# lsalzman/enet

Measured on AMD Instinct MI355X. Metric: GiB/s device-resident range-coder (de)compress, 64Ki×1200B pkts, 1/2/4/8 GPU, higher is better.
Workload: dtype u8; 1 GPU; C2 65536x1200B uniform-random, compress+decompress round trip; packets_per_gpu=65536, packet_bytes=1200, parallelism=shard1, out_cap=2N+64

## Files before the change

enet_amd/csrc/rc_dec6.hip:

```cpp


#ifndef RC_LANE_HOST_TEST
#include <hip/hip_runtime.h>
#else
#include "lane_host_shim.h"
#endif
#include <stdint.h>
#include <type_traits>

#include "rc_abi_internal.h"
#include "rc_udiv.h"
#include "rc_lane_common.h"
#include "rc_root3.h"
#include "rc_dec6_rare.h"
#include "rc_slot.h"

namespace {

#ifndef DEC6_BLOCK
#define DEC6_BLOCK 16
#endif
#ifndef DEC6_PRIO
#define DEC6_PRIO 3
#endif
#ifndef DEC6_HELP_SLEEP
#define DEC6_HELP_SLEEP 4
#endif
#ifndef DEC6_RARE_ITERS
#define DEC6_RARE_ITERS 2
#endif
constexpr uint32_t kBlock6 = DEC6_BLOCK;
constexpr uint32_t kRareIters6 = DEC6_RARE_ITERS;
constexpr uint32_t kWaveBail6 = 16;
constexpr uint32_t kStats6 = kRootStrideDec;
constexpr uint32_t kLds6 = kRootStrideDec + 256;
constexpr uint32_t kDummy6 = 256 * kTab2Rec;

DEV void bail6(const rc_workspace_dev& ws, uint32_t pkt) { bail(ws, pkt); }

DEV void reset6(uint8_t* root, uint8_t* stats, Root& R, uint32_t& rtot, double& rrt, uint32_t& order, uint32_t& a,
                uint32_t& p, uint32_t& nodes, uint32_t& nh, bool& repeat, bool& o2s, bool& e2d, uint32_t& seg0,
                uint32_t& rst, uint32_t n)
{
    root3_clear<false>(root, R);
    const uint4 z = make_uint4(0u, 0u, 0u, 0u);
#pragma unroll
    for (int i = 0; i < 16; ++i) reinterpret_cast<uint4*>(stats)[i] = z;
    rtot = 1 + 256;
    rrt = rcp64(rtot);
    order = 0; a = 0; p = 0; nodes = 1; nh = 0;
    repeat = false; o2s = false; e2d = false;
    rst = (rst | (n << (12 * (rst >> 24)))) + (1u << 24);
    seg0 = n;
}

DEV bool can_reset6(uint32_t rst, uint32_t n) { return (rst >> 24) < 2 && n < 4096; }

struct ByteSink1 {
    uint32_t acc, nb, ws;
    uint4 w, wp;
    bool pend;
    uintptr_t waddr, wpaddr, lo;
    uint32_t n, cap;
};

DEV void sink1_init(ByteSink1& o, uint8_t* p, uint32_t cap)
{
    o.lo = reinterpret_cast<uintptr_t>(p);
    o.waddr = o.lo & ~static_cast<uintptr_t>(15);
    o.wpaddr = o.waddr;
    o.ws = static_cast<uint32_t>(o.lo & 15) >> 2;
    o.nb = static_cast<uint32_t>(o.lo & 3);
    o.acc = 0;
    o.w = make_uint4(0u, 0u, 0u, 0u);
    o.wp = o.w;
    o.pend = false;
    o.n = 0;
    o.cap = cap;
}

DEV void sink1_flush(ByteSink1& o)
{
    sink_store(o.wpaddr, o.wp, o.lo, o.pend);
    o.pend = false;
}

DEV void sink1_put(ByteSink1& o, uint32_t v, bool en)
{
    o.acc |= en ? (v << (8 * o.nb)) : 0u;
    o.nb += en ? 1u : 0u;
    o.n += en ? 1u : 0u;
    const bool mv = o.nb == 4;
    o.w.x = mv ? o.w.y : o.w.x; o.w.y = mv ? o.w.z : o.w.y; o.w.z = mv ? o.w.w : o.w.z; o.w.w = mv ? o.acc : o.w.w;
    o.acc = mv ? 0u : o.acc;
    o.nb = mv ? 0u : o.nb;
    o.ws += mv ? 1u : 0u;
    const bool full = o.ws == 4;
    o.wp.x = full ? o.w.x : o.wp.x; o.wp.y = full ? o.w.y : o.wp.y;
    o.wp.z = full ? o.w.z : o.wp.z; o.wp.w = full ? o.w.w : o.wp.w;
    o.wpaddr = full ? o.waddr : o.wpaddr;
    o.pend = o.pend || full;
    o.ws = full ? 0u : o.ws;
    o.waddr += full ? 16 : 0;
}

DEV void sink1_finish(ByteSink1& o)
{
    sink1_flush(o);
    const uint32_t ws = o.ws;
    const uint32_t d[4] = {o.w.x, o.w.y, o.w.z, o.w.w};
    uint32_t q[4];
#pragma unroll
    for (uint32_t j = 0; j < 4; ++j) {
        const uint32_t k = 4 - ws + j;
        q[j] = j < ws ? (k == 0 ? d[0] : k == 1 ? d[1] : k == 2 ? d[2] : d[3]) : (j == ws ? o.acc : 0u);
    }
    sink_bytes(o.waddr, make_uint4(q[0], q[1], q[2], q[3]), 0ull, 4 * ws + o.nb, o.lo);
}

template <class Src>
DEV void decompress_one6(const rc_batch_dev& bt, const rc_workspace_dev& ws, uint32_t pkt, uint8_t* root,
                         uint8_t* stats, uint8_t* tab, uint8_t* tab2, const uint8_t* itab, Src& in,
                         const double* rtab = nullptr)
{
    constexpr bool kSlot = std::is_same<Src, SlotSrc>::value;
    const uint32_t len = bt.in_len[pkt];
    const uint32_t cap = bt.out_cap[pkt];
    if (len == 0) { bt.out_len[pkt] = 0; ws.claims[pkt] = 0; ws.dec6_resets[pkt] = 0; return; }
    ByteSink1 o;
    sink1_init(o, bt.out + bt.out_off[pkt], cap);
    uint32_t code;
    if constexpr (kSlot) {
        code = slot_init(in, bt.in + bt.in_off[pkt], len, pkt);
    } else {
        src_init(in, bt.in + bt.in_off[pkt], len);
        code = static_cast<uint32_t>(in.la >> 32);
        in.la <<= 32;
        in.na -= 4;
        src_refill(in, true);
    }
    Root R;
    root3_clear<false>(root, R);
    {
        const uint4 z = make_uint4(0u, 0u, 0u, 0u);
#pragma unroll
        for (int i = 0; i < 16; ++i) reinterpret_cast<uint4*>(stats)[i] = z;
    }
    uint32_t rtot = 1 + 256;
    double rrt = rcp64(rtot);
    uint32_t low = 0, range = ~0u;

    uint32_t order = 0, a = 0, p = 0, nodes = 1, claims = 0, x0 = 0;
    uint32_t hl[4] = {0u, 0u, 0u, 0u}, nh = 0;
    bool repeat = false;
    bool o2s = false;
    bool e2d = false;
    bool stall = false, done = false, off = false, fail = false;
    uint32_t seg0 = 0, rst = 0;

    PROF_DECL
    uint32_t s = 0;
#ifdef DEC6_STATS_PREFETCH
    uint32_t stn = 0;
    double rtn = 1.0;
#endif
    for (;;) {
        {
            uint32_t shc = 0;
            uint4 ssl = make_uint4(0u, 0u, 0u, 0u);
            if constexpr (kSlot) {
                slot_read(in, shc, ssl);
            } else {
                src_fill(in, true);
            }
            sink1_flush(o);
            const bool go = !done && !stall;
#ifdef DEC6_STATS_PREFETCH
            const uint32_t st = (go && order >= 1) ? stn : 0u;
#else
            const uint32_t sraw = stats[p];
            const uint32_t st = (go && order >= 1) ? sraw : 0u;
#endif
            const uint32_t t1 = st & 31u, d1 = t1 - (st >> 5);
            bool need = go && order >= 2 && repeat && !o2s;
            bool e2 = false;
            const bool c2s = go && order >= 2 && repeat && o2s;
            if (any_lane(c2s)) {
                const uint32_t r2 = udiv16d(range, 7u, 1.0 / 7.0);
                e2 = c2s && code - low < 5u * r2;
                need = need || (c2s && !e2);
                range = e2 ? r2 : range;
                dec_code(low, code, range, 0u, 5u, in, e2);
            }
            const bool o1 = go && !need && order >= 1 && t1 > 0;
            const uint32_t esc1 = kSubEscDelta * d1, tot1 = o1 ? esc1 + kSubDelta * t1 : 1u;
#ifdef DEC6_STATS_PREFETCH
            const uint32_t r1 = udiv16d(range, tot1, o1 ? rtn : 1.0);
#elif defined(DEC6_RCP_TAB) && !defined(RC_LANE_HOST_TEST)
            const uint32_t r1 = udiv16d(range, tot1, rtab[st]);
#else
            const uint32_t r1 = udiv16d(range, tot1, rcp64(tot1));
#endif
#ifndef DEC6_READ1
            const bool e1 = o1 && code - low < esc1 * r1;
            need = need || (o1 && !e1);
#else
            const uint32_t cd1 = udiv_lo16(code - low, r1);
            need = need || (o1 && cd1 >= esc1);
            const bool e1 = o1 && cd1 < esc1;
#endif
            need = need && !(ws.dec6_debug & 2);
            range = e1 ? r1 : range;
            dec_code(low, code, range, 0u, esc1, in, e1);
            const bool rg = go && !need;
            const uint32_t r0 = udiv16d(range, rtot, rrt);
            const uint32_t cd0 = udiv_lo16(code - low, r0);
            const bool eos = rg && cd0 < 1;
            const bool past = rg && !eos && cd0 - 1 >= rtot - 1;
            const bool sym = rg && !eos && !past;
            range = sym ? r0 : range;
            uint32_t under0 = 0, cnt0 = 0;
#ifndef DEC6_ITAB_LATE
            uint4 i0, i1;
            const uint32_t v = root3_search_inc(root, R, itab, sym ? cd0 - 1 : 0u, under0, cnt0, i0, i1);
#else
            const uint32_t v = root3_search(root, R, sym ? cd0 - 1 : 0u, under0, cnt0);
#endif
            dec_code_late(low, code, range, 1 + under0, 1 + cnt0, in, sym);
            if (sym) {
#ifndef DEC6_ITAB_LATE
                root3_add_pre(root, R, v, cnt0, i0, i1);
#else
                root3_add_inc(root, R, itab, v, cnt0);
#endif
                rtot = (rtot + kRootDelta) & 0xFFFF;
            }
            if (rare_lane(sym && (1 + cnt0 > 0xFF - 2 * kRootDelta + 1 || rtot > kTotalLimit))) {
                if (sym && (1 + cnt0 > 0xFF - 2 * kRootDelta + 1 || rtot > kTotalLimit))
                    rtot = root3_rescale<false>(root, R);
            }
            rrt = sym ? rcp64(rtot) : rrt;
            nodes += sym ? (cnt0 == 0 ? 1u : 0u) + (order >= 1 ? 1u : 0u) + (order >= 2 ? 1u : 0u) : 0u;
            const bool o1v = sym && order >= 1;
#ifndef DEC6_STATS_PREFETCH
            stats[p] = static_cast<uint8_t>(o1v ? st + 1 : sraw);
#else
            if (o1v) stats[p] = static_cast<uint8_t>(st + 1);
#endif
            const bool full = o1v && t1 >= kTabCap;
            *GPTR(uint16_t, !(o1v && !full) ? reinterpret_cast<uintptr_t>(tab2) + kDummy6 : rec_addr(tab, tab2, p, t1)) =
                static_cast<uint16_t>(a | (v << 8));
            x0 = (sym && order == 0) ? v : x0;
            const bool fl = sym && o.n >= o.cap;
            claims += (o1v && !fl) ? 1u : 0u;
            const bool rs0 = sym && nodes >= kMaxNodes;
            const bool lv = past || full || (rs0 && !can_reset6(rst, o.n + 1));
            off = off || lv;
            fail = fail || fl;
            done = done || eos || lv || fl;
            sink1_put(o, v, sym && !lv && !fl);
            a = sym ? p : a;
            p = sym ? v : p;
            order += (sym && order < 2) ? 1u : 0u;
            repeat = sym ? false : repeat;
            o2s = sym ? false : o2s;
            e2d = go ? (e2 && need) : e2d;
            stall = stall || need;
            if (rare_lane(rs0 && !done)) {
                if (rs0 && !done) reset6(root, stats, R, rtot, rrt, order, a, p, nodes, nh, repeat, o2s, e2d, seg0, rst, o.n);
            }
#ifdef DEC6_STATS_PREFETCH
            stn = stats[p];
            {
                const uint32_t nt = stn & 31u, nd1 = nt - (stn >> 5);
                rtn = rcp64(max(kSubEscDelta * nd1 + kSubDelta * nt, 1u));
            }
#endif
            PROF(0)
            if constexpr (kSlot) slot_step_end(in, ssl, shc);
            else src_adv(in);
            PROF(5)
        }
        ++s;
        if (s < kBlock6 && any_lane(!done && !stall)) continue;
        s = 0;
        for (uint32_t it = 0; it < kRareIters6 && any_lane(stall && !done); ++it) {
            const bool rs = stall && !done;
            uint32_t shc = 0;
            uint4 ssl = make_uint4(0u, 0u, 0u, 0u);
            if constexpr (kSlot) {
                slot_read(in, shc, ssl);
            } else {
                src_fill(in, true);
            }
            sink1_flush(o);
#ifdef DEC6_DRAIN
            __builtin_amdgcn_s_waitcnt(0);
#endif
            const uint32_t st = rs && order >= 1 ? stats[p] : 0u;
            const uint32_t t1 = st & 31u, d1 = t1 - (st >> 5);
            Hist6 H;
            rec_build(tab, tab2, p, rs ? t1 : 0u, hl, nh, x0, o.n - seg0, rs, H);
            const bool over = false;
            PROF(1)
#ifdef RC_PROFILE
            prof_acc[8] += 1;
            prof_acc[9] += static_cast<unsigned long long>(__builtin_popcountll(__builtin_amdgcn_ballot_w64(rs)));
#endif
            uint32_t nd = 1;
#pragma unroll
            for (uint32_t j = 1; j < 8; ++j) nd += any_lane(H.k > 4 * j) ? 1u : 0u;
            uint32_t pl[8];
            planes6(H.V, nd, pl);
            const uint32_t km = low_bits(H.k);
            const uint32_t g2 = (rs && order >= 2) ? (eqmask6(H.A, a, nd) & km & ~H.p1) : 0u;
            const uint32_t g1 = km & ~H.hit;
            const uint32_t t2 = popc(g2);
            uint32_t d2 = 0;
            {
                uint32_t rem = g2;
                while (any_lane(rem != 0)) {
                    const uint32_t j = rem ? static_cast<uint32_t>(__builtin_ctz(rem)) : 0u;
                    const uint32_t same = peq6(pl, pval6(pl, j)) & g2 & low_bits(j);
                    d2 += (rem != 0 && same == 0) ? 1u : 0u;
                    rem &= rem ? rem - 1u : 0u;
                }
            }
            int at = -1;
            uint32_t v = 0, hu = 0, hc = 0;
            bool sf = false;
            const bool c2 = rs && !over && !e2d && order >= 2 && t2 > 0;
            if (any_lane(c2)) {
                if (sub_decode6(pl, g2, t2, d2, c2, low, code, range, in, v, hu, hc, sf)) at = 2;
            }
            const bool c1 = rs && !over && !sf && at < 0 && order >= 1 && t1 > 0;
            if (any_lane(c1)) {
                if (sub_decode6(pl, g1, t1, d1, c1, low, code, range, in, v, hu, hc, sf)) at = 1;
            }
            const bool rg = rs && !over && !sf && at < 0;
            const uint32_t r0 = udiv16d(range, rtot, rrt);
            const uint32_t cd0 = udiv_lo16(code - low, r0);
            const bool eos = rg && cd0 < 1;
            const bool past = rg && !eos && cd0 - 1 >= rtot - 1;
            const bool sym0 = rg && !eos && !past;
            range = sym0 ? r0 : range;
            uint32_t under0 = 0, cnt0 = 0;
            const uint32_t v0 = root3_search(root, R, sym0 ? cd0 - 1 : 0u, under0, cnt0);
            const bool sym = sym0 || at > 0;
            v = sym0 ? v0 : v;
            dec_code(low, code, range, sym0 ? 1 + under0 : hu, sym0 ? 1 + cnt0 : hc, in, sym);
            if (sym0) {
                root3_add_inc(root, R, itab, v, cnt0);
                rtot = (rtot + kRootDelta) & 0xFFFF;
            }
            if (rare_lane(sym0 && (1 + cnt0 > 0xFF - 2 * kRootDelta + 1 || rtot > kTotalLimit))) {
                if (sym0 && (1 + cnt0 > 0xFF - 2 * kRootDelta + 1 || rtot > kTotalLimit))
                    rtot = root3_rescale<false>(root, R);
            }
            rrt = sym0 ? rcp64(rtot) : rrt;
            PROF(2)
            const uint32_t eqv = peq6(pl, v) & km;
            const bool n2 = order >= 2 && (eqv & g2) == 0;
            const bool n1 = order >= 1 && at != 2 && (eqv & g1) == 0;
            const bool nb = eqv == 0;
            nodes += sym ? (sym0 && cnt0 == 0 ? 1u : 0u) + (n2 ? 1u : 0u) + (n1 ? 1u : 0u) : 0u;
            const bool o1v = sym && order >= 1 && at != 2;
            const uint32_t nst = st + 1 + (n1 ? 0u : 32u);
            if (o1v) stats[p] = static_cast<uint8_t>(nst);
            const bool tfull = o1v && t1 >= kTabCap;
            if (o1v && !tfull)
                *GPTR(uint16_t, rec_addr(tab, tab2, p, t1)) =
                    static_cast<uint16_t>(a | (v << 8));
            claims += (sym && order >= 1 && nb && o.n < o.cap) ? 1u : 0u;
            const bool h2 = sym && at == 2;
            const uint32_t he = p | (a << 8) | (v << 16);
#pragma unroll
            for (uint32_t h = 0; h < 4; ++h) hl[h] = (h2 && nh == h) ? he : hl[h];
            const bool hfull = h2 && nh >= 4;
            nh += h2 ? 1u : 0u;
            const bool fl = sym && o.n >= o.cap;
            const bool rs0 = rs && sym && nodes >= kMaxNodes;
            const bool lv = over || sf || past || hfull || tfull || (o1v && !n1 && (st >> 5) >= 7) ||
                            (rs0 && !can_reset6(rst, o.n + 1));
            off = off || (rs && lv);
            fail = fail || (rs && fl);
            done = done || (rs && (eos || lv || fl));
            sink1_put(o, v, sym && !lv && !fl);
            a = sym ? p : a;
            p = sym ? v : p;
            order += (sym && order < 2) ? 1u : 0u;
            repeat = sym ? !nb : repeat;
            const bool one = sym && popc(eqv) == 1;
            o2s = rs ? one : o2s;
            e2d = rs ? false : e2d;
            stall = rs ? (sym && !lv && !fl && order >= 2 && repeat && !one) : stall;
            if (rare_lane(rs0 && !done)) {
                if (rs0 && !done) {
                    reset6(root, stats, R, rtot, rrt, order, a, p, nodes, nh, repeat, o2s, e2d, seg0, rst, o.n);
                    stall = false;
                }
            }
            if constexpr (kSlot) slot_step_end(in, ssl, shc);
            else src_adv(in);
            PROF(3)
        }
#ifdef DEC6_END_WAIT
        __builtin_amdgcn_s_waitcnt(0);
#endif
#ifdef DEC6_STATS_PREFETCH
        stn = stats[p];
        {
            const uint32_t nt = stn & 31u, nd1 = nt - (stn >> 5);
            rtn = rcp64(max(kSubEscDelta * nd1 + kSubDelta * nt, 1u));
        }
#endif
        const uint32_t left = static_cast<uint32_t>(__builtin_popcountll(__builtin_amdgcn_ballot_w64(off)));
        if (left >= kWaveBail6) { off = off || !done; done = true; }
        PROF(4)
        if (!any_lane(!done)) break;
    }
    PROF_FLUSH(16)
#ifndef DEC6_NO_USED_CHECK
    if constexpr (kSlot) {
        const uint32_t used = 16 * in.j + 4 * in.q - in.lo15 - in.na;
        off = off || (!fail && (used < len || used > len + 4));
    }
#endif
    if (off) { bail6(ws, pkt); ws.claims[pkt] = 0xFFFFFFFFu; return; }
    ws.dec6_resets[pkt] = rst;
    if constexpr (kSlot) ws.dec6_icks[pkt] = in.cks;
    sink1_finish(o);
    bt.out_len[pkt] = o.n;
    ws.claims[pkt] = claims | (fail ? 0x80000000u : 0u);
}

}

#ifndef RC_LANE_HOST_TEST
constexpr uint32_t kLanes6s = 256;
extern "C" __global__ __launch_bounds__(512) void rc_decompress_dec6s(rc_batch_dev b, rc_workspace_dev ws)
{
    extern __shared__ __attribute__((aligned(16))) uint8_t smem[];
    const uint32_t wave = threadIdx.x >> 6;
    const bool helper = wave >= 4;
    const uint32_t L = (wave & 3) * 64 + (threadIdx.x & 63);
    uint8_t* root = smem + L * kLds6;
    uint8_t* stats = root + kStats6;
    uint8_t* slotp = root + 256;
    uint32_t* mctl = reinterpret_cast<uint32_t*>(smem + kLanes6s * kLds6) + 2 * L;
    uint32_t* hctl = reinterpret_cast<uint32_t*>(smem + kLanes6s * kLds6 + 8 * kLanes6s) + L;
    uint8_t* itab = smem + kLanes6s * (kLds6 + 12);
    const uint32_t slot = blockIdx.x * kLanes6s + L;
    if (!helper) *reinterpret_cast<uint2*>(mctl) = make_uint2(0u, slot < b.n ? kNoPktS : kFinS);
    else *hctl = 0u;
    if (threadIdx.x < 16) root3_inc_init(itab, threadIdx.x);
    double* rtab = reinterpret_cast<double*>(itab + 512);
#ifdef DEC6_RCP_TAB
    if (threadIdx.x < 256) {
        const uint32_t t1 = threadIdx.x & 31u, r1 = threadIdx.x >> 5;
        const uint32_t tot = (t1 > 0 && r1 <= t1) ? kSubEscDelta * (t1 - r1) + kSubDelta * t1 : 1u;
        rtab[threadIdx.x] = rcp64(tot);
    }
#endif
    __syncthreads();
    if (helper) {
        SlotHelp h;
        slot_help_init(h);
#ifdef DEC6_HELP_COUNT
        uint32_t nb = 0, ni = 0;
#endif
        for (;;) {
            bool fin = false;
            const bool busy = slot_help_iter(b, mctl, hctl, slotp, h, ws.dec6_hcks, ws.n_cap, fin);
#ifdef DEC6_HELP_COUNT
            nb += busy ? 1u : 0u;
            ni += busy ? 0u : 1u;
#endif
            if (fin) break;
            if (!busy) __builtin_amdgcn_s_sleep(DEC6_HELP_SLEEP);
        }
#ifdef DEC6_HELP_COUNT
        if ((threadIdx.x & 63) == 0) { atomicAdd(&ws.counters[5], nb); atomicAdd(&ws.counters[6], ni); }
#endif
        return;
    }
    uint8_t* tab = static_cast<uint8_t*>(ws.dec6_pool) + static_cast<size_t>(slot) * kTab1;
    uint8_t* tab2 = static_cast<uint8_t*>(ws.dec6_pool) + static_cast<size_t>(ws.lane_slots) * kTab1 +
                    static_cast<size_t>(slot) * kTab2;
    const uint32_t* order = ws.order && !ws.bins[RC_LEN_BINS] ? ws.order : nullptr;
    __builtin_amdgcn_s_setprio(DEC6_PRIO);
    SlotSrc in;
    in.gen = 0; in.mctl = mctl; in.hctl = hctl; in.slot = slotp;
    for (uint32_t i = slot; i < b.n; i += gridDim.x * kLanes6s) {
        const uint32_t pkt = order ? order[i] : i;
        decompress_one6(b, ws, pkt, root, stats, tab, tab2, itab, in, rtab);
    }
    mctl[1] = kFinS;
}

constexpr uint32_t kVerifyWaves = 4;
constexpr uint32_t kVerifyBlocksPerCu = 10;
constexpr uint32_t kVerDw = 8;

DEV uint32_t vhead_load(const rc_batch_dev& b, const rc_workspace_dev& ws, uint32_t k, uint32_t l)
{
    const uint32_t* src = l == 0 ? ws.claims + k
                        : l == 1 ? b.out_len + k
                        : l < 4 ? reinterpret_cast<const uint32_t*>(b.out_off + k) + (l - 2)
                        : l == 4 ? ws.dec6_resets + k
                        : l == 5 ? ws.dec6_icks + k
                        : l == 6 ? ws.dec6_hcks + k
                                 : ws.dec6_hcks + ws.n_cap + k;
    return (k < b.n && l < 8) ? *src : 0u;
}


struct VHead {
    uint32_t cl, n, rst, off, nd;
    uintptr_t lo, sb;
    bool skip, fast, cks;
};

DEV VHead vhead_get(const rc_batch_dev& b, uint32_t k, uint32_t hv)
{
    VHead h;
    h.cl = __shfl(hv, 0);
    h.n = __shfl(hv, 1);
    const uint64_t oo = static_cast<uint64_t>(static_cast<uint32_t>(__shfl(hv, 2))) |
                        static_cast<uint64_t>(static_cast<uint32_t>(__shfl(hv, 3))) << 32;
    h.rst = __shfl(hv, 4);
    h.cks = cks_agree(__shfl(hv, 5), __shfl(hv, 6), __shfl(hv, 7));
    h.skip = k >= b.n || h.cl == 0xFFFFFFFFu;
    h.lo = reinterpret_cast<uintptr_t>(b.out) + oo;
    h.sb = h.lo & ~static_cast<uintptr_t>(3);
    h.off = static_cast<uint32_t>(h.lo - h.sb);
    h.nd = (h.off + h.n + 3) >> 2;
    h.fast = !h.skip && (h.rst >> 24) == 0 && h.nd <= 64 * kVerDw;
    return h;
}

DEV void vdata_load(const VHead& h, uint32_t l, uint32_t (&w)[kVerDw])
{
    const uint32_t* p = reinterpret_cast<const uint32_t*>(h.sb);
#pragma unroll
    for (uint32_t r = 0; r < kVerDw; ++r) {
        const uint32_t c = 64 * r + l;
        w[r] = (h.fast && c < h.nd) ? p[c] : 0u;
    }
}

DEV void vresult(const rc_batch_dev& b, const rc_workspace_dev& ws, uint32_t k, uint32_t cl, uint32_t cnt, bool ck,
                 uint32_t l)
{
    for (int sft = 32; sft >= 1; sft >>= 1) cnt += static_cast<uint32_t>(__shfl_xor(static_cast<int>(cnt), sft));
    const uint32_t want = cl & 0x7FFFFFFFu;
    const bool ok = cnt == want && ck && !(ws.dec6_debug & 1);
    if (l == 0 && !ok) {
        const uint32_t i = atomicAdd(&ws.counters[3], 1u);
        ws.enc2_list[i] = k;
        if (!ck) atomicAdd(&ws.counters[7], 1u);
    }
    if (l == 0 && ok && (cl >> 31)) b.out_len[k] = 0;
}

DEV void vclear(uint4* set4, uint32_t l)
{
#pragma unroll
    for (uint32_t i = 0; i < 512 / 64; ++i) set4[i * 64 + l] = make_uint4(0u, 0u, 0u, 0u);
}

DEV void verify_fast(const rc_batch_dev& b, const rc_workspace_dev& ws, uint32_t k, const VHead& h,
                     const uint32_t (&w)[kVerDw], uint4* set4, uint32_t l)
{
    uint32_t* set = reinterpret_cast<uint32_t*>(set4);
    vclear(set4, l);
    uint32_t cnt = 0, last = 0;
#pragma unroll
    for (uint32_t r = 0; r < kVerDw; ++r) {
        if (64 * r >= h.nd) break;
        const uint32_t up = static_cast<uint32_t>(__shfl_up(static_cast<int>(w[r]), 1));
        const uint32_t pw = l ? up : last;
        last = static_cast<uint32_t>(__shfl(static_cast<int>(w[r]), 63));
        const uint32_t c = 64 * r + l;
#pragma unroll
        for (uint32_t t = 0; t < 4; ++t) {
            const uint32_t x = (w[r] >> (8 * t)) & 0xFFu;
            const uint32_t pv = t ? (w[r] >> (8 * t - 8)) & 0xFFu : pw >> 24;
            const uint32_t pos = 4 * c + t - h.off;
            const bool in = pos >= 1 && pos < h.n;
            const uint32_t bg = (pv << 8) | x, bit = 1u << (bg & 31);
#ifdef VERIFY_RETURNS
            const uint32_t old = atomicOr(&set[in ? bg >> 5 : l], in ? bit : 0u);
            cnt += (in && !(old & bit)) ? 1u : 0u;
#else
            atomicOr(&set[in ? bg >> 5 : l], in ? bit : 0u);
#endif
        }
    }
#ifndef VERIFY_RETURNS
    __builtin_amdgcn_fence(__ATOMIC_SEQ_CST, "wavefront");
    __builtin_amdgcn_wave_barrier();
#pragma unroll
    for (uint32_t i = 0; i < 512 / 64; ++i) {
        const uint4 q = set4[i * 64 + l];
        cnt += static_cast<uint32_t>(__builtin_popcount(q.x) + __builtin_popcount(q.y) + __builtin_popcount(q.z) +
                                     __builtin_popcount(q.w));
    }
#endif
    vresult(b, ws, k, h.cl, cnt, h.cks, l);
}

DEV void verify_slow(const rc_batch_dev& b, const rc_workspace_dev& ws, uint32_t pkt, uint4* set4, uint32_t l)
{
    uint32_t* set = reinterpret_cast<uint32_t*>(set4);
    {
        const uint32_t cl = ws.claims[pkt];
        const uint32_t n = b.out_len[pkt];
        const uintptr_t lo = reinterpret_cast<uintptr_t>(b.out + b.out_off[pkt]);
        const uint32_t rst = ws.dec6_resets[pkt], nseg = (rst >> 24) + 1;
        uint32_t cnt = 0;
        for (uint32_t sg = 0; sg < nseg; ++sg) {
            const uint32_t s0 = sg ? (rst >> (12 * (sg - 1))) & 0xFFFu : 0u;
            const uint32_t s1 = sg + 1 < nseg ? (rst >> (12 * sg)) & 0xFFFu : n;
#pragma unroll
            for (uint32_t i = 0; i < 512 / 64; ++i) set4[i * 64 + l] = make_uint4(0u, 0u, 0u, 0u);
            __builtin_amdgcn_wave_barrier();
            const uintptr_t slo = lo + s0;
            const uintptr_t sb = slo & ~static_cast<uintptr_t>(15);
            const uint32_t m = s1 > s0 ? s1 - s0 : 0u;
            const uint32_t chunks = m > 1 ? static_cast<uint32_t>((slo + m - sb + 15) >> 4) : 0u;
            for (uint32_t c = l; c < chunks; c += 64) {
                const uintptr_t a = sb + 16 * c;
                const uint4 w = *reinterpret_cast<const uint4*>(a);
                uint32_t prev = a > slo ? *reinterpret_cast<const uint8_t*>(a - 1) : 0u;
                const uint32_t d[4] = {w.x, w.y, w.z, w.w};
#pragma unroll
                for (uint32_t t = 0; t < 16; ++t) {
                    const uint32_t x = (d[t >> 2] >> (8 * (t & 3))) & 0xFFu;
                    const uintptr_t at = a + t;
                    if (at > slo && at < slo + m) {
                        const uint32_t bg = (prev << 8) | x;
                        atomicOr(&set[bg >> 5], 1u << (bg & 31));
                    }
                    prev = x;
                }
            }
            __builtin_amdgcn_wave_barrier();
            uint32_t sc = 0;
#pragma unroll
            for (uint32_t i = 0; i < 512 / 64; ++i) {
                const uint4 q = set4[i * 64 + l];
                sc += static_cast<uint32_t>(__builtin_popcount(q.x) + __builtin_popcount(q.y) +
                                            __builtin_popcount(q.z) + __builtin_popcount(q.w));
            }
            cnt += sc;
            __builtin_amdgcn_wave_barrier();
        }
        vresult(b, ws, pkt, cl, cnt, cks_agree(ws.dec6_icks[pkt], ws.dec6_hcks[pkt], ws.dec6_hcks[ws.n_cap + pkt]), l);
    }
}

DEV void verify_one(const rc_batch_dev& b, const rc_workspace_dev& ws, uint32_t k, const VHead& h,
                    const uint32_t (&w)[kVerDw], uint4* set4, uint32_t l)
{
    if (h.skip) return;
    if (h.fast) verify_fast(b, ws, k, h, w, set4, l);
    else verify_slow(b, ws, k, set4, l);
    __builtin_amdgcn_wave_barrier();
}

extern "C" __global__ __launch_bounds__(256) __attribute__((amdgpu_waves_per_eu(5)))
void rc_dec6_verify(rc_batch_dev b, rc_workspace_dev ws)
{
    __shared__ uint4 bits[kVerifyWaves][512];
    const uint32_t wave = threadIdx.x >> 6, l = threadIdx.x & 63;
    uint4* set4 = bits[wave];
    const uint32_t stride = gridDim.x * kVerifyWaves;
    uint32_t k = blockIdx.x * kVerifyWaves + wave;
    if (k >= b.n) return;
    uint32_t wa[kVerDw], wb[kVerDw];
    uint32_t hva = vhead_load(b, ws, k, l);
    VHead ha = vhead_get(b, k, hva), hb;
    vdata_load(ha, l, wa);
    uint32_t hvb = vhead_load(b, ws, k + stride, l);
    for (;;) {
        hb = vhead_get(b, k + stride, hvb);
        vdata_load(hb, l, wb);
        hva = vhead_load(b, ws, k + 2 * stride, l);
        verify_one(b, ws, k, ha, wa, set4, l);
        k += stride;
        if (k >= b.n) break;
        ha = vhead_get(b, k + stride, hva);
        vdata_load(ha, l, wa);
        hvb = vhead_load(b, ws, k + 2 * stride, l);
        verify_one(b, ws, k, hb, wb, set4, l);
        k += stride;
        if (k >= b.n) break;
    }
}

extern "C" int rc_hip_dec6_verify_launch(const rc_batch_dev* b, const rc_workspace_dev* ws, void* stream)
{
    hipStream_t st = static_cast<hipStream_t>(stream);
    const uint32_t vb = (b->n + kVerifyWaves - 1) / kVerifyWaves;
    static const char* vb_env = getenv("ENET_RC_VERIFY_BPC");
    const uint32_t bpc = vb_env && atoi(vb_env) > 0 ? static_cast<uint32_t>(atoi(vb_env)) : kVerifyBlocksPerCu;
    const uint32_t cap = (ws->cus ? ws->cus : 256u) * bpc;
    hipLaunchKernelGGL(rc_dec6_verify, dim3(vb < cap ? vb : cap), dim3(256), 0, st, *b, *ws);
    return static_cast<int>(hipGetLastError());
}

extern "C" int rc_hip_dec6_launch(const rc_batch_dev* b, const rc_workspace_dev* ws, uint32_t blocks, void* stream)
{
    hipStream_t st = static_cast<hipStream_t>(stream);
    if (ws->lane_active != 64) return static_cast<int>(hipErrorInvalidValue);
#ifdef DEC6_RCP_TAB
    const size_t lds = static_cast<size_t>(kLanes6s) * (kLds6 + 12) + 512 + 2048;
#else
    const size_t lds = static_cast<size_t>(kLanes6s) * (kLds6 + 12) + 512;
#endif
    hipLaunchKernelGGL(rc_decompress_dec6s, dim3(blocks), dim3(512), lds, st, *b, *ws);
    const hipError_t e = hipGetLastError();
    if (e != hipSuccess) return static_cast<int>(e);
    return rc_hip_dec6_verify_launch(b, ws, stream);
}
#endif
```

enet_amd/csrc/rc_dec6_rare.h:

```cpp
#pragma once

namespace {

DEV uint32_t eq01(uint32_t x, uint32_t y)
{
    const uint32_t z = x ^ y;
    const uint32_t t = ((z & 0x7F7F7F7Fu) + 0x7F7F7F7Fu) | z;
    return (~t >> 7) & 0x01010101u;
}

DEV uint32_t gather4(uint32_t e) { return (e | (e >> 7) | (e >> 14) | (e >> 21)) & 0xFu; }

DEV uint32_t popc(uint32_t x) { return static_cast<uint32_t>(__builtin_popcount(x)); }
DEV uint32_t low_bits(uint32_t n) { return n >= 32 ? 0xFFFFFFFFu : ((1u << n) - 1u); }

DEV void bail(const rc_workspace_dev& ws, uint32_t pkt)
{
    const uint32_t slot = atomicAdd(&ws.counters[3], 1u);
    ws.enc2_list[slot] = pkt;
}

constexpr uint32_t kTab1 = 256 * 16;
constexpr uint32_t kTab2Rec = 48;
constexpr uint32_t kTab2 = 256 * kTab2Rec + 128;
constexpr uint32_t kTabCap = 28;

struct Hist6 { uint32_t A[8], V[8]; uint32_t p1, hit, k; };

DEV uint4 hload16(uintptr_t a)
{
#ifndef RC_LANE_HOST_TEST
    const uint64_t lo = __hip_atomic_load(GPTRC(uint64_t, a), __ATOMIC_RELAXED, __HIP_MEMORY_SCOPE_AGENT);
    const uint64_t hi = __hip_atomic_load(GPTRC(uint64_t, a + 8), __ATOMIC_RELAXED, __HIP_MEMORY_SCOPE_AGENT);
    return make_uint4(static_cast<uint32_t>(lo), static_cast<uint32_t>(lo >> 32), static_cast<uint32_t>(hi),
                      static_cast<uint32_t>(hi >> 32));
#else
    return gload16(a);
#endif
}

DEV uint32_t eqmask6(const uint32_t* X, uint32_t u, uint32_t nd)
{
    const uint32_t ur = u * 0x01010101u;
    uint32_t m = 0;
#pragma unroll
    for (uint32_t d = 0; d < 8; ++d)
        if (d < nd) m |= gather4(eq01(X[d], ur)) << (4 * d);
    return m;
}

DEV uintptr_t rec_addr(const uint8_t* tab, const uint8_t* tab2, uint32_t p, uint32_t t)
{
    return t < 8 ? reinterpret_cast<uintptr_t>(tab) + 16 * p + 2 * t
                 : reinterpret_cast<uintptr_t>(tab2) + kTab2Rec * p + 2 * (t - 8);
}

DEV void rec_load(const uint8_t* tab, const uint8_t* tab2, uint32_t p, uint32_t t1, bool en, uint4& r1, uint4& r2,
                  uint4& r3, uint4& r4)
{
    const uint4 z = make_uint4(0u, 0u, 0u, 0u);
    r1 = z; r2 = z; r3 = z; r4 = z;
    const uintptr_t b2 = reinterpret_cast<uintptr_t>(tab2) + kTab2Rec * p;
    if (en) r1 = hload16(reinterpret_cast<uintptr_t>(tab) + 16 * p);
    if (en && t1 > 8) {
        r2 = hload16(b2);
        r3 = hload16(b2 + 16);
    }
    if (rare_lane(en && t1 > 24)) {
        if (en && t1 > 24) r4 = hload16(b2 + 32);
    }
}

DEV void rec_fill(const uint4& r1, const uint4& r2, const uint4& r3, const uint4& r4, uint32_t p, uint32_t t1,
                  const uint32_t* hl, uint32_t nh, uint32_t x0, uint32_t n, Hist6& H)
{
    H.A[0] = bperm(r1.y, r1.x, 0x06040200u); H.V[0] = bperm(r1.y, r1.x, 0x07050301u);
    H.A[1] = bperm(r1.w, r1.z, 0x06040200u); H.V[1] = bperm(r1.w, r1.z, 0x07050301u);
    H.A[2] = bperm(r2.y, r2.x, 0x06040200u); H.V[2] = bperm(r2.y, r2.x, 0x07050301u);
    H.A[3] = bperm(r2.w, r2.z, 0x06040200u); H.V[3] = bperm(r2.w, r2.z, 0x07050301u);
    H.A[4] = bperm(r3.y, r3.x, 0x06040200u); H.V[4] = bperm(r3.y, r3.x, 0x07050301u);
    H.A[5] = bperm(r3.w, r3.z, 0x06040200u); H.V[5] = bperm(r3.w, r3.z, 0x07050301u);
    H.A[6] = bperm(r4.y, r4.x, 0x06040200u); H.V[6] = bperm(r4.y, r4.x, 0x07050301u);
    H.A[7] = 0u; H.V[7] = 0u;
    H.p1 = (p == x0 && t1 > 0 && n >= 2) ? 1u : 0u;
    H.hit = 0u;
    uint32_t k = t1;
    if (any_lane(nh > 0))
#pragma unroll
    for (uint32_t h = 0; h < 4; ++h) {
        const bool mine = h < nh && (hl[h] & 0xFFu) == p;
        const uint32_t ks = 8 * (k & 3);
#pragma unroll
        for (uint32_t d = 0; d < 8; ++d) {
            const bool here = mine && (k >> 2) == d;
            H.A[d] = here ? ((H.A[d] & ~(0xFFu << ks)) | (((hl[h] >> 8) & 0xFFu) << ks)) : H.A[d];
            H.V[d] = here ? ((H.V[d] & ~(0xFFu << ks)) | (((hl[h] >> 16) & 0xFFu) << ks)) : H.V[d];
        }
        H.hit |= mine ? (1u << k) : 0u;
        k += mine ? 1u : 0u;
    }
    H.k = k;
}

DEV void rec_build(const uint8_t* tab, const uint8_t* tab2, uint32_t p, uint32_t t1, const uint32_t* hl, uint32_t nh,
                   uint32_t x0, uint32_t n, bool en, Hist6& H)
{
    uint4 r1, r2, r3, r4;
    rec_load(tab, tab2, p, t1, en, r1, r2, r3, r4);
    rec_fill(r1, r2, r3, r4, p, t1, hl, nh, x0, n, H);
}

DEV void planes6(const uint32_t* V, uint32_t nd, uint32_t* pl)
{
#pragma unroll
    for (uint32_t b = 0; b < 8; ++b) {
        uint32_t m = 0;
#pragma unroll
        for (uint32_t d = 0; d < 8; ++d)
            if (d < nd) m |= dot4((V[d] >> b) & 0x01010101u, 0x08040201u, 0u) << (4 * d);
        pl[b] = m;
    }
}

DEV uint32_t peq6(const uint32_t* pl, uint32_t u)
{
    uint32_t m = 0xFFFFFFFFu;
#pragma unroll
    for (uint32_t b = 0; b < 8; ++b) m &= ((u >> b) & 1u) ? pl[b] : ~pl[b];
    return m;
}

DEV uint32_t pselect6(const uint32_t* pl, uint32_t g, uint32_t q, uint32_t& lt, uint32_t& eq)
{
    uint32_t cand = g, below = 0, u = 0;
#pragma unroll
    for (int b = 7; b >= 0; --b) {
        const uint32_t zeros = cand & ~pl[b];
        const uint32_t nz = popc(zeros);
        const bool one = q >= below + nz;
        below += one ? nz : 0u;
        cand = one ? (cand & pl[b]) : zeros;
        u |= one ? (1u << b) : 0u;
    }
    lt = below;
    eq = popc(cand);
    return u;
}

DEV uint32_t pval6(const uint32_t* pl, uint32_t j)
{
    uint32_t u = 0;
#pragma unroll
    for (uint32_t b = 0; b < 8; ++b) u |= ((pl[b] >> j) & 1u) << b;
    return u;
}

template <class Src>
DEV bool sub_decode6(const uint32_t* pl, uint32_t g, uint32_t t, uint32_t d, bool en, uint32_t& low,
                     uint32_t& code, uint32_t& range, Src& in, uint32_t& v, uint32_t& under, uint32_t& count,
                     bool& fail)
{
    const uint32_t esc = kSubEscDelta * d, tot = en ? esc + kSubDelta * t : 1u;
    const uint32_t r1 = udiv16d(range, tot, rcp64(tot));
    const uint32_t cd = udiv_lo16(code - low, r1);
    range = en ? r1 : range;
    const bool e = en && cd < esc;
    dec_code(low, code, range, 0u, esc, in, e);
    const bool hit = en && !e;
    fail = fail || (hit && cd - esc >= kSubDelta * t);
    const bool sel = hit && cd - esc < kSubDelta * t;
    if (any_lane(sel)) {
        uint32_t lt, eq;
        const uint32_t u = pselect6(pl, g, sel ? (cd - esc) >> 1 : 0u, lt, eq);
        under = sel ? esc + kSubDelta * lt : under;
        count = sel ? kSubDelta * eq : count;
        v = sel ? u : v;
    }
    return sel;
}

}
```

Before: 23.86 GiB/s.

## Prefetch stalled-lane history records during tail decode steps; skip idle rare-path work

Moves the per-symbol decode body into an always-inlined lambda. It adds an optional tail mode, DEC6_TAIL, that issues the history-record loads for stalled lanes, runs one to three more fast steps, then completes the records, so load latency overlaps useful work. By default the rare escape loop now skips the root-model division, search and update when no lane needs them. rec_fill also skips each history-hit merge iteration when no lane matches. The tail prefetch is off by default (DEC6_TAIL=0), so only the wave-uniform skips run, and they add extra branch and vote overhead.

```diff
diff --git a/enet_amd/csrc/rc_dec6.hip b/enet_amd/csrc/rc_dec6.hip
--- a/enet_amd/csrc/rc_dec6.hip
+++ b/enet_amd/csrc/rc_dec6.hip
@@ -29,7 +29,16 @@
 #ifndef DEC6_RARE_ITERS
 #define DEC6_RARE_ITERS 2
 #endif
+#ifndef DEC6_TAIL
+#define DEC6_TAIL 0
+#endif
+#if DEC6_TAIL < 0 || DEC6_TAIL > 3
+#error "DEC6_TAIL: 0-3"
+#endif
+#define DEC6_STEP_INLINE __attribute__((always_inline))
 constexpr uint32_t kBlock6 = DEC6_BLOCK;
+constexpr uint32_t kTail6 = DEC6_TAIL;
+static_assert(kTail6 < kBlock6, "DEC6_TAIL: below DEC6_BLOCK");
 constexpr uint32_t kRareIters6 = DEC6_RARE_ITERS;
 constexpr uint32_t kWaveBail6 = 16;
 constexpr uint32_t kStats6 = kRootStrideDec;
@@ -121,7 +130,7 @@
 template <class Src>
 DEV void decompress_one6(const rc_batch_dev& bt, const rc_workspace_dev& ws, uint32_t pkt, uint8_t* root,
                          uint8_t* stats, uint8_t* tab, uint8_t* tab2, const uint8_t* itab, Src& in,
-                         const double* rtab = nullptr)
+                         const double* rtab = nullptr, const uint8_t* dum = nullptr)
 {
     constexpr bool kSlot = std::is_same<Src, SlotSrc>::value;
     const uint32_t len = bt.in_len[pkt];
@@ -159,131 +168,165 @@
     uint32_t seg0 = 0, rst = 0;
 
     PROF_DECL
-    uint32_t s = 0;
 #ifdef DEC6_STATS_PREFETCH
     uint32_t stn = 0;
     double rtn = 1.0;
 #endif
+    auto step = [&]() DEC6_STEP_INLINE {
+        uint32_t shc = 0;
+        uint4 ssl = make_uint4(0u, 0u, 0u, 0u);
+        if constexpr (kSlot) {
+            slot_read(in, shc, ssl);
+        } else {
+            src_fill(in, true);
+        }
+        sink1_flush(o);
+        const bool go = !done && !stall;
+#ifdef DEC6_STATS_PREFETCH
+        const uint32_t st = (go && order >= 1) ? stn : 0u;
+#else
+        const uint32_t sraw = stats[p];
+        const uint32_t st = (go && order >= 1) ? sraw : 0u;
+#endif
+        const uint32_t t1 = st & 31u, d1 = t1 - (st >> 5);
+        bool need = go && order >= 2 && repeat && !o2s;
+        bool e2 = false;
+        const bool c2s = go && order >= 2 && repeat && o2s;
+        if (any_lane(c2s)) {
+            const uint32_t r2 = udiv16d(range, 7u, 1.0 / 7.0);
+            e2 = c2s && code - low < 5u * r2;
+            need = need || (c2s && !e2);
+            range = e2 ? r2 : range;
+            dec_code(low, code, range, 0u, 5u, in, e2);
+        }
+        const bool o1 = go && !need && order >= 1 && t1 > 0;
+        const uint32_t esc1 = kSubEscDelta * d1, tot1 = o1 ? esc1 + kSubDelta * t1 : 1u;
+#ifdef DEC6_STATS_PREFETCH
+        const uint32_t r1 = udiv16d(range, tot1, o1 ? rtn : 1.0);
+#elif defined(DEC6_RCP_TAB) && !defined(RC_LANE_HOST_TEST)
+        const uint32_t r1 = udiv16d(range, tot1, rtab[st]);
+#else
+        const uint32_t r1 = udiv16d(range, tot1, rcp64(tot1));
+#endif
+#ifndef DEC6_READ1
+        const bool e1 = o1 && code - low < esc1 * r1;
+        need = need || (o1 && !e1);
+#else
+        const uint32_t cd1 = udiv_lo16(code - low, r1);
+        need = need || (o1 && cd1 >= esc1);
+        const bool e1 = o1 && cd1 < esc1;
+#endif
+        need = need && !(ws.dec6_debug & 2);
+        range = e1 ? r1 : range;
+        dec_code(low, code, range, 0u, esc1, in, e1);
+        const bool rg = go && !need;
+        const uint32_t r0 = udiv16d(range, rtot, rrt);
+        const uint32_t cd0 = udiv_lo16(code - low, r0);
+        const bool eos = rg && cd0 < 1;
+        const bool past = rg && !eos && cd0 - 1 >= rtot - 1;
+        const bool sym = rg && !eos && !past;
+        range = sym ? r0 : range;
+        uint32_t under0 = 0, cnt0 = 0;
+#ifndef DEC6_ITAB_LATE
+        uint4 i0, i1;
+        const uint32_t v = root3_search_inc(root, R, itab, sym ? cd0 - 1 : 0u, under0, cnt0, i0, i1);
+#else
+        const uint32_t v = root3_search(root, R, sym ? cd0 - 1 : 0u, under0, cnt0);
+#endif
+        dec_code_late(low, code, range, 1 + under0, 1 + cnt0, in, sym);
+        if (sym) {
+#ifndef DEC6_ITAB_LATE
+            root3_add_pre(root, R, v, cnt0, i0, i1);
+#else
+            root3_add_inc(root, R, itab, v, cnt0);
+#endif
+            rtot = (rtot + kRootDelta) & 0xFFFF;
+        }
+        if (rare_lane(sym && (1 + cnt0 > 0xFF - 2 * kRootDelta + 1 || rtot > kTotalLimit))) {
+            if (sym && (1 + cnt0 > 0xFF - 2 * kRootDelta + 1 || rtot > kTotalLimit))
+                rtot = root3_rescale<false>(root, R);
+        }
+        rrt = sym ? rcp64(rtot) : rrt;
+        nodes += sym ? (cnt0 == 0 ? 1u : 0u) + (order >= 1 ? 1u : 0u) + (order >= 2 ? 1u : 0u) : 0u;
+        const bool o1v = sym && order >= 1;
+#ifndef DEC6_STATS_PREFETCH
+        stats[p] = static_cast<uint8_t>(o1v ? st + 1 : sraw);
+#else
+        if (o1v) stats[p] = static_cast<uint8_t>(st + 1);
+#endif
+        const bool full = o1v && t1 >= kTabCap;
+        *GPTR(uint16_t, !(o1v && !full) ? reinterpret_cast<uintptr_t>(tab2) + kDummy6 : rec_addr(tab, tab2, p, t1)) =
+            static_cast<uint16_t>(a | (v << 8));
+        x0 = (sym && order == 0) ? v : x0;
+        const bool fl = sym && o.n >= o.cap;
+        claims += (o1v && !fl) ? 1u : 0u;
+        const bool rs0 = sym && nodes >= kMaxNodes;
+        const bool lv = past || full || (rs0 && !can_reset6(rst, o.n + 1));
+        off = off || lv;
+        fail = fail || fl;
+        done = done || eos || lv || fl;
+        sink1_put(o, v, sym && !lv && !fl);
+        a = sym ? p : a;
+        p = sym ? v : p;
+        order += (sym && order < 2) ? 1u : 0u;
+        repeat = sym ? false : repeat;
+        o2s = sym ? false : o2s;
+        e2d = go ? (e2 && need) : e2d;
+        stall = stall || need;
+        if (rare_lane(rs0 && !done)) {
+            if (rs0 && !done) reset6(root, stats, R, rtot, rrt, order, a, p, nodes, nh, repeat, o2s, e2d, seg0, rst, o.n);
+        }
+#ifdef DEC6_STATS_PREFETCH
+        stn = stats[p];
+        {
+            const uint32_t nt = stn & 31u, nd1 = nt - (stn >> 5);
+            rtn = rcp64(max(kSubEscDelta * nd1 + kSubDelta * nt, 1u));
+        }
+#endif
+        PROF(0)
+        if constexpr (kSlot) slot_step_end(in, ssl, shc);
+        else src_adv(in);
+        PROF(5)
+    };
+    uint32_t s = 0;
     for (;;) {
-        {
-            uint32_t shc = 0;
-            uint4 ssl = make_uint4(0u, 0u, 0u, 0u);
-            if constexpr (kSlot) {
-                slot_read(in, shc, ssl);
-            } else {
-                src_fill(in, true);
-            }
-            sink1_flush(o);
-            const bool go = !done && !stall;
-#ifdef DEC6_STATS_PREFETCH
-            const uint32_t st = (go && order >= 1) ? stn : 0u;
-#else
-            const uint32_t sraw = stats[p];
-            const uint32_t st = (go && order >= 1) ? sraw : 0u;
-#endif
-            const uint32_t t1 = st & 31u, d1 = t1 - (st >> 5);
-            bool need = go && order >= 2 && repeat && !o2s;
-            bool e2 = false;
-            const bool c2s = go && order >= 2 && repeat && o2s;
-            if (any_lane(c2s)) {
-                const uint32_t r2 = udiv16d(range, 7u, 1.0 / 7.0);
-                e2 = c2s && code - low < 5u * r2;
-                need = need || (c2s && !e2);
-                range = e2 ? r2 : range;
-                dec_code(low, code, range, 0u, 5u, in, e2);
-            }
-            const bool o1 = go && !need && order >= 1 && t1 > 0;
-            const uint32_t esc1 = kSubEscDelta * d1, tot1 = o1 ? esc1 + kSubDelta * t1 : 1u;
-#ifdef DEC6_STATS_PREFETCH
-            const uint32_t r1 = udiv16d(range, tot1, o1 ? rtn : 1.0);
-#elif defined(DEC6_RCP_TAB) && !defined(RC_LANE_HOST_TEST)
-            const uint32_t r1 = udiv16d(range, tot1, rtab[st]);
-#else
-            const uint32_t r1 = udiv16d(range, tot1, rcp64(tot1));
-#endif
-#ifndef DEC6_READ1
-            const bool e1 = o1 && code - low < esc1 * r1;
-            need = need || (o1 && !e1);
-#else
-            const uint32_t cd1 = udiv_lo16(code - low, r1);
-            need = need || (o1 && cd1 >= esc1);
-            const bool e1 = o1 && cd1 < esc1;
-#endif
-            need = need && !(ws.dec6_debug & 2);
-            range = e1 ? r1 : range;
-            dec_code(low, code, range, 0u, esc1, in, e1);
-            const bool rg = go && !need;
-            const uint32_t r0 = udiv16d(range, rtot, rrt);
-            const uint32_t cd0 = udiv_lo16(code - low, r0);
-            const bool eos = rg && cd0 < 1;
-            const bool past = rg && !eos && cd0 - 1 >= rtot - 1;
-            const bool sym = rg && !eos && !past;
-            range = sym ? r0 : range;
-            uint32_t under0 = 0, cnt0 = 0;
-#ifndef DEC6_ITAB_LATE
-            uint4 i0, i1;
-            const uint32_t v = root3_search_inc(root, R, itab, sym ? cd0 - 1 : 0u, under0, cnt0, i0, i1);
-#else
-            const uint32_t v = root3_search(root, R, sym ? cd0 - 1 : 0u, under0, cnt0);
-#endif
-            dec_code_late(low, code, range, 1 + under0, 1 + cnt0, in, sym);
-            if (sym) {
-#ifndef DEC6_ITAB_LATE
-                root3_add_pre(root, R, v, cnt0, i0, i1);
-#else
-                root3_add_inc(root, R, itab, v, cnt0);
-#endif
-                rtot = (rtot + kRootDelta) & 0xFFFF;
-            }
-            if (rare_lane(sym && (1 + cnt0 > 0xFF - 2 * kRootDelta + 1 || rtot > kTotalLimit))) {
-                if (sym && (1 + cnt0 > 0xFF - 2 * kRootDelta + 1 || rtot > kTotalLimit))
-                    rtot = root3_rescale<false>(root, R);
-            }
-            rrt = sym ? rcp64(rtot) : rrt;
-            nodes += sym ? (cnt0 == 0 ? 1u : 0u) + (order >= 1 ? 1u : 0u) + (order >= 2 ? 1u : 0u) : 0u;
-            const bool o1v = sym && order >= 1;
-#ifndef DEC6_STATS_PREFETCH
-            stats[p] = static_cast<uint8_t>(o1v ? st + 1 : sraw);
-#else
-            if (o1v) stats[p] = static_cast<uint8_t>(st + 1);
-#endif
-            const bool full = o1v && t1 >= kTabCap;
-            *GPTR(uint16_t, !(o1v && !full) ? reinterpret_cast<uintptr_t>(tab2) + kDummy6 : rec_addr(tab, tab2, p, t1)) =
-                static_cast<uint16_t>(a | (v << 8));
-            x0 = (sym && order == 0) ? v : x0;
-            const bool fl = sym && o.n >= o.cap;
-            claims += (o1v && !fl) ? 1u : 0u;
-            const bool rs0 = sym && nodes >= kMaxNodes;
-            const bool lv = past || full || (rs0 && !can_reset6(rst, o.n + 1));
-            off = off || lv;
-            fail = fail || fl;
-            done = done || eos || lv || fl;
-            sink1_put(o, v, sym && !lv && !fl);
-            a = sym ? p : a;
-            p = sym ? v : p;
-            order += (sym && order < 2) ? 1u : 0u;
-            repeat = sym ? false : repeat;
-            o2s = sym ? false : o2s;
-            e2d = go ? (e2 && need) : e2d;
-            stall = stall || need;
-            if (rare_lane(rs0 && !done)) {
-                if (rs0 && !done) reset6(root, stats, R, rtot, rrt, order, a, p, nodes, nh, repeat, o2s, e2d, seg0, rst, o.n);
-            }
-#ifdef DEC6_STATS_PREFETCH
-            stn = stats[p];
-            {
-                const uint32_t nt = stn & 31u, nd1 = nt - (stn >> 5);
-                rtn = rcp64(max(kSubEscDelta * nd1 + kSubDelta * nt, 1u));
-            }
-#endif
-            PROF(0)
-            if constexpr (kSlot) slot_step_end(in, ssl, shc);
-            else src_adv(in);
-            PROF(5)
-        }
+#if DEC6_TAIL == 0
+        step();
         ++s;
         if (s < kBlock6 && any_lane(!done && !stall)) continue;
         s = 0;
+        Hist6 H;
+        const bool pre = false;
+#else
+        s = 0;
+        bool can;
+        do {
+            step();
+            ++s;
+            can = any_lane(!done && !stall);
+        } while (s < kBlock6 - kTail6 && can);
+        Hist6 H;
+        bool pre = false;
+        if (can) {
+            const bool pf = stall && !done;
+            const uint32_t pst = pf && order >= 1 ? stats[p] : 0u;
+            uint4 r1, r2, r3, r4;
+            rec_request(tab, tab2, dum ? dum : tab2 + kDummy6, p, pst & 31u, pf, r1, r2, r3);
+            step();
+#if DEC6_TAIL > 1
+            step();
+#endif
+#if DEC6_TAIL > 2
+            step();
+#endif
+            const bool sv = stall && !done;
+            const uint32_t sst = sv && order >= 1 ? stats[p] : 0u;
+            rec_late(tab, tab2, p, sst & 31u, sv && !pf, r1, r2, r3);
+            rec_take(tab2, p, sst & 31u, sv, r1, r2, r3, r4);
+            rec_fill(r1, r2, r3, r4, p, sst & 31u, hl, nh, x0, o.n - seg0, sv, H);
+            pre = true;
+        }
+#endif
         for (uint32_t it = 0; it < kRareIters6 && any_lane(stall && !done); ++it) {
             const bool rs = stall && !done;
             uint32_t shc = 0;
@@ -299,8 +342,7 @@
 #endif
             const uint32_t st = rs && order >= 1 ? stats[p] : 0u;
             const uint32_t t1 = st & 31u, d1 = t1 - (st >> 5);
-            Hist6 H;
-            rec_build(tab, tab2, p, rs ? t1 : 0u, hl, nh, x0, o.n - seg0, rs, H);
+            if (!pre || it > 0) rec_build(tab, tab2, p, rs ? t1 : 0u, hl, nh, x0, o.n - seg0, rs, H);
             const bool over = false;
             PROF(1)
 #ifdef RC_PROFILE
@@ -338,26 +380,37 @@
                 if (sub_decode6(pl, g1, t1, d1, c1, low, code, range, in, v, hu, hc, sf)) at = 1;
             }
             const bool rg = rs && !over && !sf && at < 0;
-            const uint32_t r0 = udiv16d(range, rtot, rrt);
-            const uint32_t cd0 = udiv_lo16(code - low, r0);
-            const bool eos = rg && cd0 < 1;
-            const bool past = rg && !eos && cd0 - 1 >= rtot - 1;
-            const bool sym0 = rg && !eos && !past;
-            range = sym0 ? r0 : range;
+            bool eos = false, past = false, sym0 = false;
             uint32_t under0 = 0, cnt0 = 0;
-            const uint32_t v0 = root3_search(root, R, sym0 ? cd0 - 1 : 0u, under0, cnt0);
+#ifndef DEC6_ROOT_ALWAYS
+            if (any_lane(rg))
+#endif
+            {
+                const uint32_t r0 = udiv16d(range, rtot, rrt);
+                const uint32_t cd0 = udiv_lo16(code - low, r0);
+                eos = rg && cd0 < 1;
+                past = rg && !eos && cd0 - 1 >= rtot - 1;
+                sym0 = rg && !eos && !past;
+                range = sym0 ? r0 : range;
+                const uint32_t v0 = root3_search(root, R, sym0 ? cd0 - 1 : 0u, under0, cnt0);
+                v = sym0 ? v0 : v;
+            }
             const bool sym = sym0 || at > 0;
-            v = sym0 ? v0 : v;
             dec_code(low, code, range, sym0 ? 1 + under0 : hu, sym0 ? 1 + cnt0 : hc, in, sym);
-            if (sym0) {
-                root3_add_inc(root, R, itab, v, cnt0);
-                rtot = (rtot + kRootDelta) & 0xFFFF;
-            }
-            if (rare_lane(sym0 && (1 + cnt0 > 0xFF - 2 * kRootDelta + 1 || rtot > kTotalLimit))) {
-                if (sym0 && (1 + cnt0 > 0xFF - 2 * kRootDelta + 1 || rtot > kTotalLimit))
-                    rtot = root3_rescale<false>(root, R);
-            }
-            rrt = sym0 ? rcp64(rtot) : rrt;
+#ifndef DEC6_ROOT_ALWAYS
+            if (any_lane(sym0))
+#endif
+            {
+                if (sym0) {
+                    root3_add_inc(root, R, itab, v, cnt0);
+                    rtot = (rtot + kRootDelta) & 0xFFFF;
+                }
+                if (rare_lane(sym0 && (1 + cnt0 > 0xFF - 2 * kRootDelta + 1 || rtot > kTotalLimit))) {
+                    if (sym0 && (1 + cnt0 > 0xFF - 2 * kRootDelta + 1 || rtot > kTotalLimit))
+                        rtot = root3_rescale<false>(root, R);
+                }
+                rrt = sym0 ? rcp64(rtot) : rrt;
+            }
             PROF(2)
             const uint32_t eqv = peq6(pl, v) & km;
             const bool n2 = order >= 2 && (eqv & g2) == 0;
@@ -487,13 +540,14 @@
     uint8_t* tab = static_cast<uint8_t*>(ws.dec6_pool) + static_cast<size_t>(slot) * kTab1;
     uint8_t* tab2 = static_cast<uint8_t*>(ws.dec6_pool) + static_cast<size_t>(ws.lane_slots) * kTab1 +
                     static_cast<size_t>(slot) * kTab2;
+    const uint8_t* dum = static_cast<uint8_t*>(ws.dec6_pool) + static_cast<size_t>(ws.lane_slots) * kTab1 + kDummy6;
     const uint32_t* order = ws.order && !ws.bins[RC_LEN_BINS] ? ws.order : nullptr;
     __builtin_amdgcn_s_setprio(DEC6_PRIO);
     SlotSrc in;
     in.gen = 0; in.mctl = mctl; in.hctl = hctl; in.slot = slotp;
     for (uint32_t i = slot; i < b.n; i += gridDim.x * kLanes6s) {
         const uint32_t pkt = order ? order[i] : i;
-        decompress_one6(b, ws, pkt, root, stats, tab, tab2, itab, in, rtab);
+        decompress_one6(b, ws, pkt, root, stats, tab, tab2, itab, in, rtab, dum);
     }
     mctl[1] = kFinS;
 }
diff --git a/enet_amd/csrc/rc_dec6_rare.h b/enet_amd/csrc/rc_dec6_rare.h
--- a/enet_amd/csrc/rc_dec6_rare.h
+++ b/enet_amd/csrc/rc_dec6_rare.h
@@ -71,8 +71,61 @@
     }
 }
 
+
+DEV void rec_settle(uint4& r)
+{
+#ifndef RC_LANE_HOST_TEST
+    asm volatile("" : "+v"(r.x), "+v"(r.y), "+v"(r.z), "+v"(r.w));
+#endif
+}
+
+DEV uint4 sel16(bool c, const uint4& x, const uint4& y)
+{
+    return make_uint4(c ? x.x : y.x, c ? x.y : y.y, c ? x.z : y.z, c ? x.w : y.w);
+}
+
+DEV void rec_request(const uint8_t* tab, const uint8_t* tab2, const uint8_t* dum, uint32_t p, uint32_t t1, bool en,
+                     uint4& r1, uint4& r2, uint4& r3)
+{
+    const uintptr_t d = reinterpret_cast<uintptr_t>(dum);
+    const uintptr_t b2 = reinterpret_cast<uintptr_t>(tab2) + kTab2Rec * p;
+    const bool big = en && t1 > 8;
+    r1 = hload16(en ? reinterpret_cast<uintptr_t>(tab) + 16 * p : d);
+    r2 = hload16(big ? b2 : d);
+    r3 = hload16(big ? b2 + 16 : d + 16);
+}
+
+DEV void rec_late(const uint8_t* tab, const uint8_t* tab2, uint32_t p, uint32_t t1, bool en, uint4& r1, uint4& r2,
+                  uint4& r3)
+{
+    if (any_lane(en)) {
+        const uintptr_t b2 = reinterpret_cast<uintptr_t>(tab2) + kTab2Rec * p;
+        uint4 l1 = r1, l2 = r2, l3 = r3;
+        if (en) l1 = hload16(reinterpret_cast<uintptr_t>(tab) + 16 * p);
+        if (en && t1 > 8) {
+            l2 = hload16(b2);
+            l3 = hload16(b2 + 16);
+        }
+        rec_settle(l1); rec_settle(l2); rec_settle(l3);
+        r1 = l1; r2 = l2; r3 = l3;
+    }
+}
+
+DEV void rec_take(const uint8_t* tab2, uint32_t p, uint32_t t1, bool en, uint4& r1, uint4& r2, uint4& r3, uint4& r4)
+{
+    const uint4 z = make_uint4(0u, 0u, 0u, 0u);
+    r1 = sel16(en, r1, z);
+    r2 = sel16(en && t1 > 8, r2, z);
+    r3 = sel16(en && t1 > 8, r3, z);
+    r4 = z;
+    if (rare_lane(en && t1 > 24)) {
+        if (en && t1 > 24) r4 = hload16(reinterpret_cast<uintptr_t>(tab2) + kTab2Rec * p + 32);
+        rec_settle(r4);
+    }
+}
+
 DEV void rec_fill(const uint4& r1, const uint4& r2, const uint4& r3, const uint4& r4, uint32_t p, uint32_t t1,
-                  const uint32_t* hl, uint32_t nh, uint32_t x0, uint32_t n, Hist6& H)
+                  const uint32_t* hl, uint32_t nh, uint32_t x0, uint32_t n, bool en, Hist6& H)
 {
     H.A[0] = bperm(r1.y, r1.x, 0x06040200u); H.V[0] = bperm(r1.y, r1.x, 0x07050301u);
     H.A[1] = bperm(r1.w, r1.z, 0x06040200u); H.V[1] = bperm(r1.w, r1.z, 0x07050301u);
@@ -85,10 +138,17 @@
     H.p1 = (p == x0 && t1 > 0 && n >= 2) ? 1u : 0u;
     H.hit = 0u;
     uint32_t k = t1;
+#ifdef DEC6_HITS_ALWAYS
     if (any_lane(nh > 0))
+#endif
 #pragma unroll
     for (uint32_t h = 0; h < 4; ++h) {
+#ifdef DEC6_HITS_ALWAYS
         const bool mine = h < nh && (hl[h] & 0xFFu) == p;
+#else
+        const bool mine = en && h < nh && (hl[h] & 0xFFu) == p;
+        if (!any_lane(mine)) continue;
+#endif
         const uint32_t ks = 8 * (k & 3);
 #pragma unroll
         for (uint32_t d = 0; d < 8; ++d) {
@@ -107,7 +167,7 @@
 {
     uint4 r1, r2, r3, r4;
     rec_load(tab, tab2, p, t1, en, r1, r2, r3, r4);
-    rec_fill(r1, r2, r3, r4, p, t1, hl, nh, x0, n, H);
+    rec_fill(r1, r2, r3, r4, p, t1, hl, nh, x0, n, en, H);
 }
 
 DEV void planes6(const uint32_t* V, uint32_t nd, uint32_t* pl)
```

New measurement: 24.14 GiB/s, median of 6. +1.2%, better.
